# seaweedfs/seaweedfs

Measured on NVIDIA H100. Metric: rs10_4_encode_input_GBps, higher is better.
Workload: dtype u8

## Files before the change

### seaweedfs_b200/build.py

```python
from __future__ import annotations

import hashlib
import os
import shutil
import subprocess
import sys

HERE = os.path.dirname(os.path.abspath(__file__))
CSRC = os.path.join(HERE, "csrc")
GEN = os.path.join(CSRC, "generated")
LIB = os.path.join(HERE, "libswec.so")
ROOT = os.path.dirname(HERE)

SOURCES = ["kernels.cu", "aot_recon.cu", "needles.cu", "damage.cu", "engine.cc", "host_seam.cc", "ec_files.cc", "ec_index.cc", "ec_volume.cc", "volume_format.cc", "staging.cc",
           "jit.cc", "codegen.cc", "gf256.cc"]
HEADERS = ["apply_params.h", "device_common.cuh", "kernels.h", "engine.h", "host_seam.h", "gf256.h", "codegen.h", "io_pool.h", "mini_json.h",
           "volume_format.h", "needle_format.h", "needles.h", "damage.h", "staging.h", os.path.join(ROOT, "include", "swec.h")]
NVCC_FLAGS = ["-gencode", "arch=compute_90a,code=sm_90a", "-O3", "-lineinfo", "-std=c++17",
              "-Xcompiler", "-fPIC,-Wall,-Wno-unused-function", "-cudart", "static"]


def _nvcc() -> str:
    for cand in (os.environ.get("NVCC"), shutil.which("nvcc"), "/usr/local/cuda/bin/nvcc"):
        if cand and os.path.exists(cand):
            return cand
    raise RuntimeError("nvcc not found — libswec.so cannot be built (there is no CPU fallback)")


def _run(cmd: list[str], **kw) -> None:
    r = subprocess.run(cmd, stdout=subprocess.PIPE, stderr=subprocess.STDOUT, text=True, **kw)
    if r.returncode != 0:
        sys.stderr.write(r.stdout)
        raise RuntimeError("command failed: " + " ".join(cmd))


def _stamp() -> str:
    h = hashlib.sha256()
    paths = [os.path.join(CSRC, s) for s in SOURCES + ["codegen_main.cc"]] + \
            [p if os.path.isabs(p) else os.path.join(CSRC, p) for p in HEADERS] + [os.path.abspath(__file__)]
    for p in paths:
        with open(p, "rb") as f:
            h.update(f.read())
    h.update(os.environ.get("SWEC_EXTRA_NVCC_FLAGS", "").encode())
    h.update(os.environ.get("SWEC_CODEGEN_FLAGS", "").encode())
    return h.hexdigest()


def generate() -> None:
    os.makedirs(GEN, exist_ok=True)
    tool = os.path.join(GEN, "swec_codegen")
    _run(["g++", "-O2", "-std=c++17", "-o", tool] +
         [os.path.join(CSRC, s) for s in ("codegen_main.cc", "codegen.cc", "gf256.cc")])
    gen_flags = os.environ.get("SWEC_CODEGEN_FLAGS", "").split()
    out = subprocess.run([tool, "--rs", "10", "4", "--name", "Rs10x4Encode"] + gen_flags, check=True,
                         stdout=subprocess.PIPE, stderr=subprocess.DEVNULL, text=True).stdout
    with open(os.path.join(GEN, "gen_rs10x4_encode.inc"), "w") as f:
        f.write(out)
    with open(os.path.join(GEN, "gen_rs10x4_encode_lp.inc"), "w") as f:
        f.write(out.replace("struct Rs10x4Encode ", "struct Rs10x4EncodeLP "))
    for emit, name in (("structs", "gen_aot_recon.inc"), ("keys", "gen_aot_recon_keys.inc")):
        text = subprocess.run([tool, "--aot-recon", "10", "4", "--emit", emit] +
                              [f for f in gen_flags if f == "--share-powers"], check=True,
                              stdout=subprocess.PIPE, text=True).stdout
        with open(os.path.join(GEN, name), "w") as f:
            f.write(text)
    text = []
    for name in ("apply_params.h", "device_common.cuh"):
        with open(os.path.join(CSRC, name)) as f:
            for line in f:
                if line.startswith("#pragma once") or line.startswith('#include "apply_params.h"'):
                    continue
                text.append(line)
    with open(os.path.join(GEN, "device_common_src.inc"), "w") as f:
        f.write('R"SWECSRC(' + "".join(text) + ')SWECSRC"\n')


def build(force: bool = False, verbose: bool = False) -> str:
    stamp_path = os.path.join(GEN, "build.stamp")
    stamp = _stamp()
    if not force and os.path.exists(LIB) and os.path.exists(stamp_path):
        with open(stamp_path) as f:
            if f.read().strip() == stamp:
                return LIB
    generate()
    extra = os.environ.get("SWEC_EXTRA_NVCC_FLAGS", "").split()
    from concurrent.futures import ThreadPoolExecutor
    objdir = os.path.join(GEN, "obj")
    os.makedirs(objdir, exist_ok=True)
    common = [_nvcc()] + NVCC_FLAGS + extra + ["-I", CSRC, "-I", GEN]
    objs = [os.path.join(objdir, os.path.splitext(src)[0] + ".o") for src in SOURCES]

    def compile_one(pair):
        src, obj = pair
        cmd = common + ["-c", os.path.join(CSRC, src), "-o", obj]
        if verbose:
            print(" ".join(cmd))
        _run(cmd)
    with ThreadPoolExecutor(max_workers=min(len(SOURCES), os.cpu_count() or 2)) as ex:
        list(ex.map(compile_one, zip(SOURCES, objs)))
    cmd = common + ["-shared", "-o", LIB] + objs + ["-ldl", "-lpthread"]
    if verbose:
        print(" ".join(cmd))
    _run(cmd)
    with open(stamp_path, "w") as f:
        f.write(stamp)
    return LIB


if __name__ == "__main__":
    print(build(force="--force" in sys.argv, verbose=True))
```

### seaweedfs_b200/csrc/aot_recon.cu

```cuda
#include <cuda_runtime.h>

#include <atomic>
#include <cstring>

#ifndef SWEC_XT_VARIANT
#define SWEC_XT_VARIANT 0
#endif
#include "device_common.cuh"

namespace swec_aot_boost {
#include "gen_aot_recon.inc"
}
#undef SWEC_XT1A
#undef SWEC_XT1B
#define SWEC_XT1A(a, s) swec_xt1_v<2>((a), (s))
#define SWEC_XT1B(a, s) swec_xt1_v<2>((a), (s))
namespace swec_aot_lowpower {
#include "gen_aot_recon.inc"
}
#undef SWEC_XT1A
#undef SWEC_XT1B
#define SWEC_XT1A(a, s) swec_xt1_v<SWEC_XT_VARIANT>((a), (s))
#define SWEC_XT1B(a, s) swec_xt1_v<SWEC_XT_VARIANT>((a), (s))
#include "gen_aot_recon_keys.inc"
#include "kernels.h"

namespace swec {

constexpr int kAotThreads = 512, kAotUnroll = 2;

template <class Combiner>
__global__ void __launch_bounds__(kAotThreads) swec_aot_recon(const __grid_constant__ SwecApplyParams p) {
    swec_horner_body<Combiner, false, kAotUnroll>(p);
}

int aot_recon_find(int r, int k, const unsigned char* coef) {
    for (int i = 0; i < SWEC_AOT_RECON_COUNT; i++)
        if (kAotReconKeys[i].r == r && kAotReconKeys[i].k == k && memcmp(kAotReconKeys[i].c, coef, size_t(r) * size_t(k)) == 0)
            return i;
    return -1;
}

int aot_recon_count() { return SWEC_AOT_RECON_COUNT; }

static std::atomic<unsigned long long> g_aot_launches{0};
unsigned long long aot_recon_launches() { return g_aot_launches.load(); }

cudaError_t launch_aot_recon(int idx, const SwecApplyParams& p, cudaStream_t s) {
    if (p.nvec == 0) return cudaSuccess;
    if (idx < 0 || idx >= SWEC_AOT_RECON_COUNT) return cudaErrorInvalidValue;
    int sms = 132, dev = 0;
    cudaGetDevice(&dev);
    cudaDeviceGetAttribute(&sms, cudaDevAttrMultiProcessorCount, dev);
    const u64 per_cta = u64(kAotThreads) * kAotUnroll;
    const u64 need = (p.nvec + per_cta - 1) / per_cta;
    const u64 cap = u64(sms) * (kAotReconKeys[idx].r >= 3 ? 1 : 2);
    const unsigned grid = unsigned(need < cap ? need : cap);
    const bool lp = low_power_now();
    note_kernel_work(double(p.nvec) * 16.0 * double(kAotReconKeys[idx].k + kAotReconKeys[idx].r) / 3.0e12 * 1e3);
    g_kernel_launches++;
    g_aot_launches++;
    switch (idx) {
#define SWEC_AOT_CASE(I)                                                                              \
    case I:                                                                                           \
        if (lp) swec_aot_recon<swec_aot_lowpower::SwecAotRecon##I><<<grid, kAotThreads, 0, s>>>(p);     \
        else swec_aot_recon<swec_aot_boost::SwecAotRecon##I><<<grid, kAotThreads, 0, s>>>(p);           \
        break;
        SWEC_AOT_RECON_FOREACH(SWEC_AOT_CASE)
#undef SWEC_AOT_CASE
        default: return cudaErrorInvalidValue;
    }
    return cudaGetLastError();
}

}
```

### seaweedfs_b200/csrc/codegen_main.cc

```cpp
#include <cstdio>
#include <cstdlib>
#include <cstring>
#include <string>

#include <vector>

#include "codegen.h"

static std::vector<swec::Matrix> aot_recon_matrices(int k, int m) {
    const swec::Matrix gen = swec::rs_generator(k, m);
    std::vector<swec::Matrix> out;
    auto add = [&](const std::vector<int>& lost) {
        std::vector<uint8_t> present(size_t(k + m), 1);
        for (int i : lost) present[size_t(i)] = 0;
        std::vector<int> in, outs;
        swec::Matrix fused;
        if (swec::rs_reconstruct_plan(gen, k, present.data(), false, &in, &outs, &fused)) out.push_back(fused);
    };
    for (int i = 0; i < k + m; i++) add({i});
    std::vector<int> worst;
    for (int i = 0; i < m && i < k; i++) worst.push_back(i);
    add(worst);
    return out;
}

int main(int argc, char** argv) {
    swec::CodegenOptions opt;
    swec::Matrix rows;
    std::string name = "SwecGen";
    int aot_k = 0, aot_m = 0;
    bool search_basis = false;
    double step_cost = 5.0;
    std::string emit = "structs";
    for (int a = 1; a < argc; a++) {
        if (!strcmp(argv[a], "--aot-recon") && a + 2 < argc) {
            aot_k = atoi(argv[a + 1]);
            aot_m = atoi(argv[a + 2]);
            a += 2;
            continue;
        }
        if (!strcmp(argv[a], "--emit") && a + 1 < argc) {
            emit = argv[++a];
            continue;
        }
        if (!strcmp(argv[a], "--share-powers")) { opt.share_powers = true; continue; }
        if (!strcmp(argv[a], "--search-basis")) { search_basis = true; continue; }
        if (!strcmp(argv[a], "--step-cost") && a + 1 < argc) { step_cost = atof(argv[++a]); continue; }
        if (!strcmp(argv[a], "--no-basis")) opt.optimise_basis = false;
        else if (!strcmp(argv[a], "--no-cse")) opt.extract_common = false;
        else if (!strcmp(argv[a], "--name") && a + 1 < argc) name = argv[++a];
        else if (!strcmp(argv[a], "--rs") && a + 2 < argc) {
            const int k = atoi(argv[a + 1]), m = atoi(argv[a + 2]);
            a += 2;
            swec::Matrix gen = swec::rs_generator(k, m);
            rows = swec::Matrix(m, k);
            for (int p = 0; p < m; p++)
                for (int i = 0; i < k; i++) rows.at(p, i) = gen.at(k + p, i);
        } else if (!strcmp(argv[a], "--rows") && a + 2 < argc) {
            const int r = atoi(argv[a + 1]), k = atoi(argv[a + 2]);
            a += 2;
            rows = swec::Matrix(r, k);
            for (int i = 0; i < r * k && a + 1 < argc; i++) rows.v[size_t(i)] = uint8_t(atoi(argv[++a]));
        } else {
            fprintf(stderr, "usage: %s [--no-basis] [--no-cse] (--rs K M | --rows R K c...)\n", argv[0]);
            return 2;
        }
    }
    if (aot_k > 0) {
        const std::vector<swec::Matrix> mats = aot_recon_matrices(aot_k, aot_m);
        if (emit == "structs") {
            for (size_t i = 0; i < mats.size(); i++)
                fputs(swec::generate_combine(mats[i], "SwecAotRecon" + std::to_string(i), opt, nullptr).c_str(), stdout);
            return 0;
        }
        printf("// generated by seaweedfs_b200/csrc/codegen_main.cc --aot-recon %d %d --emit keys — do not edit\n", aot_k, aot_m);
        printf("#define SWEC_AOT_RECON_COUNT %zu\n#define SWEC_AOT_RECON_FOREACH(X)", mats.size());
        for (size_t i = 0; i < mats.size(); i++) printf(" X(%zu)", i);
        printf("\nstatic const struct { int r, k; unsigned char c[%d]; } kAotReconKeys[SWEC_AOT_RECON_COUNT] = {\n", aot_m * aot_k);
        for (const swec::Matrix& mx : mats) {
            printf("    {%d, %d, {", mx.rows, mx.cols);
            for (size_t j = 0; j < mx.v.size(); j++) printf("%s%d", j ? "," : "", int(mx.v[j]));
            printf("}},\n");
        }
        printf("};\n");
        return 0;
    }
    if (rows.rows == 0) return 2;
    if (search_basis && rows.rows >= 2 && rows.rows <= 4) {
        const int R = rows.rows;
        const unsigned ncomb = (1u << R) - 1;
        std::vector<unsigned> cur(static_cast<size_t>(R)), best;
        std::vector<int> idx(static_cast<size_t>(R));
        for (int i = 0; i < R; i++) idx[size_t(i)] = i + 1;
        double best_cost = 1e30;
        int tried = 0;
        for (;;) {
            for (int i = 0; i < R; i++) cur[size_t(i)] = unsigned(idx[size_t(i)]);
            swec::CodegenOptions o = opt;
            o.basis = cur;
            swec::CodegenStats cs;
            swec::generate_combine(rows, name, o, &cs);
            const double c = step_cost * cs.xtime_steps + cs.xor_ops;
            tried++;
            if (c < best_cost - 1e-9) { best_cost = c; best = cur; }
            int i = R - 1;
            while (i >= 0 && idx[size_t(i)] == int(ncomb) - (R - 1 - i)) i--;
            if (i < 0) break;
            idx[size_t(i)]++;
            for (int j = i + 1; j < R; j++) idx[size_t(j)] = idx[size_t(j - 1)] + 1;
        }
        opt.basis = best;
        fprintf(stderr, "search-basis: %d bases tried, best cost %.1f, masks", tried, best_cost);
        for (unsigned m : best) fprintf(stderr, " %u", m);
        fprintf(stderr, "\n");
    }
    swec::CodegenStats st;
    fputs(swec::generate_combine(rows, name, opt, &st).c_str(), stdout);
    return 0;
}
```

### seaweedfs_b200/csrc/device_common.cuh

```cuda
#pragma once

#include "apply_params.h"

__device__ __forceinline__ u32 swec_x3(u32 a, u32 b, u32 c) {
    u32 r;
    asm("lop3.b32 %0, %1, %2, %3, 0x96;" : "=r"(r) : "r"(a), "r"(b), "r"(c));
    return r;
}
#define SWEC_X2(a, b) ((a) ^ (b))
#define SWEC_X3(a, b, c) swec_x3((a), (b), (c))

template <int V>
__device__ __forceinline__ u32 swec_xt1_v(u32 a, u32 s) {
    if (V == 2) {
        u32 mask, a2, u, r;
        asm("prmt.b32 %0, %1, 0, 0xba98;" : "=r"(mask) : "r"(a));
        asm("mul.lo.u32 %0, %1, 2;" : "=r"(a2) : "r"(a));
        asm("lop3.b32 %0, %1, 0xfefefefe, %2, 0x6a;" : "=r"(u) : "r"(a2), "r"(s));
        asm("lop3.b32 %0, %1, 0x1d1d1d1d, %2, 0x6a;" : "=r"(r) : "r"(mask), "r"(u));
        return r;
    }
    const u32 hi = a & 0x80808080u;
    if (V == 1) {
        const u32 m = (hi >> 7) * 0x1du;
        const u32 b2 = (a ^ hi) << 1;
        return swec_x3(b2, m, s);
    }
    u32 m, a2, b2;
    asm("mul.hi.u32 %0, %1, 0x3a000000;" : "=r"(m) : "r"(hi));
    asm("mul.lo.u32 %0, %1, 2;" : "=r"(a2) : "r"(a));
    asm("mad.lo.u32 %0, %1, 0xfffffffe, %2;" : "=r"(b2) : "r"(hi), "r"(a2));
    return swec_x3(b2, m, s);
}
#if SWEC_XT_VARIANT == 3
#define SWEC_XT1A(a, s) swec_xt1_v<0>((a), (s))
#define SWEC_XT1B(a, s) swec_xt1_v<2>((a), (s))
#else
#define SWEC_XT1A(a, s) swec_xt1_v<SWEC_XT_VARIANT>((a), (s))
#define SWEC_XT1B(a, s) swec_xt1_v<SWEC_XT_VARIANT>((a), (s))
#endif
#define SWEC_XT0A(a) SWEC_XT1A((a), 0u)
#define SWEC_XT0B(a) SWEC_XT1B((a), 0u)

#ifndef SWEC_LD_POLICY
#define SWEC_LD_POLICY 0
#endif
__device__ __forceinline__ uint4 swec_ldg_stream(const u8* p) {
    uint4 r;
#if SWEC_LD_POLICY == 1
    asm volatile("ld.global.nc.L1::no_allocate.L2::256B.v4.u32 {%0, %1, %2, %3}, [%4];"
#elif SWEC_LD_POLICY == 2
    asm volatile("ld.global.nc.v4.u32 {%0, %1, %2, %3}, [%4];"
#elif SWEC_LD_POLICY == 3
    asm volatile("ld.global.nc.L1::no_allocate.v4.u32 {%0, %1, %2, %3}, [%4];"
#else
    asm volatile("ld.global.nc.L1::no_allocate.L2::128B.v4.u32 {%0, %1, %2, %3}, [%4];"
#endif
                 : "=r"(r.x), "=r"(r.y), "=r"(r.z), "=r"(r.w)
                 : "l"(p));
    return r;
}
__device__ __forceinline__ void swec_stg_stream(u8* p, const uint4& v) {
#if defined(SWEC_ST_POLICY) && SWEC_ST_POLICY == 1
    asm volatile("st.global.v4.u32 [%0], {%1, %2, %3, %4};" ::"l"(p), "r"(v.x), "r"(v.y), "r"(v.z), "r"(v.w)
                 : "memory");
#else
    asm volatile("st.global.cs.v4.u32 [%0], {%1, %2, %3, %4};" ::"l"(p), "r"(v.x), "r"(v.y), "r"(v.z), "r"(v.w)
                 : "memory");
#endif
}

template <class Combiner>
__device__ __forceinline__ void swec_combine_vec(const uint4 (&d)[Combiner::K], uint4 (&o)[Combiner::R]) {
    constexpr int K = Combiner::K, R = Combiner::R;
    u32 x[K], y[R];
#pragma unroll
    for (int i = 0; i < K; i++) x[i] = d[i].x;
    Combiner::combine(x, y);
#pragma unroll
    for (int r = 0; r < R; r++) o[r].x = y[r];
#pragma unroll
    for (int i = 0; i < K; i++) x[i] = d[i].y;
    Combiner::combine(x, y);
#pragma unroll
    for (int r = 0; r < R; r++) o[r].y = y[r];
#pragma unroll
    for (int i = 0; i < K; i++) x[i] = d[i].z;
    Combiner::combine(x, y);
#pragma unroll
    for (int r = 0; r < R; r++) o[r].z = y[r];
#pragma unroll
    for (int i = 0; i < K; i++) x[i] = d[i].w;
    Combiner::combine(x, y);
#pragma unroll
    for (int r = 0; r < R; r++) o[r].w = y[r];
}

template <class Combiner, bool BLOCKED, int UNROLL = 1>
__device__ __forceinline__ void swec_horner_body(const SwecApplyParams& p) {
    constexpr int K = Combiner::K, R = Combiner::R;
    auto in_offset = [&](u64 vv) -> u64 {
        u64 ioff = vv << 4;
        if (BLOCKED) {
            const u64 row = p.block_shift >= 0 ? (vv >> p.block_shift) : (vv / p.block_vecs);
            ioff += row * p.row_extra;
        }
        return ioff;
    };
    const u64 tile = (u64)blockDim.x * UNROLL;
    const u64 stride = (u64)gridDim.x * tile;
    for (u64 base = (u64)blockIdx.x * tile; base < p.nvec; base += stride) {
        uint4 d[UNROLL][K];
        bool live[UNROLL];
#pragma unroll
        for (int u = 0; u < UNROLL; u++) {
            const u64 v = base + (u64)u * blockDim.x + threadIdx.x;
            live[u] = v < p.nvec;
            if (live[u]) {
                const u64 ioff = in_offset(v);
#pragma unroll
                for (int i = 0; i < K; i++) d[u][i] = swec_ldg_stream(p.in[i] + ioff);
            }
        }
#pragma unroll
        for (int u = 0; u < UNROLL; u++) {
            if (live[u]) {
                uint4 o[R];
                swec_combine_vec<Combiner>(d[u], o);
                const u64 off = (base + (u64)u * blockDim.x + threadIdx.x) << 4;
#pragma unroll
                for (int r = 0; r < R; r++) swec_stg_stream(p.out[r] + off, o[r]);
            }
        }
    }
}
```

### seaweedfs_b200/csrc/jit.cc

```cpp
#include <dlfcn.h>
#include <fcntl.h>
#include <nvrtc.h>
#include <sys/stat.h>
#include <unistd.h>

#include <atomic>
#include <cstdlib>
#include <cstring>
#include <chrono>
#include <condition_variable>
#include <deque>
#include <map>
#include <mutex>
#include <thread>

#include "codegen.h"
#include "engine.h"

namespace swec {

static const char kDeviceCommonSrc[] =
#include "device_common_src.inc"
    ;

struct JitKernel {
    int threads = 256, unroll = 1;
    cudaLibrary_t lib = nullptr;
    cudaKernel_t flat = nullptr, blocked = nullptr;
    CodegenStats stats;
};

namespace {

struct Nvrtc {
    void* handle = nullptr;
    decltype(&nvrtcCreateProgram) create = nullptr;
    decltype(&nvrtcCompileProgram) compile = nullptr;
    decltype(&nvrtcGetCUBINSize) cubin_size = nullptr;
    decltype(&nvrtcGetCUBIN) cubin = nullptr;
    decltype(&nvrtcGetProgramLogSize) log_size = nullptr;
    decltype(&nvrtcGetProgramLog) log = nullptr;
    decltype(&nvrtcDestroyProgram) destroy = nullptr;
    bool ok = false;
};

Nvrtc& nvrtc() {
    static Nvrtc n = [] {
        Nvrtc r;
        if (getenv("SWEC_NO_JIT")) return r;
        const char* names[] = {"libnvrtc.so.12", "/usr/local/cuda/lib64/libnvrtc.so.12", "libnvrtc.so",
                               "/usr/local/cuda/lib64/libnvrtc.so"};
        for (const char* nm : names) {
            r.handle = dlopen(nm, RTLD_NOW | RTLD_LOCAL);
            if (r.handle) break;
        }
        if (!r.handle) return r;
#define SWEC_SYM(field, name) r.field = reinterpret_cast<decltype(r.field)>(dlsym(r.handle, name))
        SWEC_SYM(create, "nvrtcCreateProgram");
        SWEC_SYM(compile, "nvrtcCompileProgram");
        SWEC_SYM(cubin_size, "nvrtcGetCUBINSize");
        SWEC_SYM(cubin, "nvrtcGetCUBIN");
        SWEC_SYM(log_size, "nvrtcGetProgramLogSize");
        SWEC_SYM(log, "nvrtcGetProgramLog");
        SWEC_SYM(destroy, "nvrtcDestroyProgram");
#undef SWEC_SYM
        r.ok = r.create && r.compile && r.cubin_size && r.cubin && r.log_size && r.log && r.destroy;
        return r;
    }();
    return n;
}

struct JitEntry {
    enum State { kCold, kQueued, kCompiling, kReady, kFailed } state = kCold;
    int uses = 0;
    std::shared_ptr<JitKernel> kernel;
};
struct JitRequest {
    Matrix rows;
    std::vector<uint8_t> key;
    int threads, unroll, device, variant;
    bool share_powers;
};
struct JitGlobal {
    std::mutex mu;
    std::condition_variable cv;
    std::map<std::vector<uint8_t>, JitEntry> cache;
    std::deque<JitRequest> queue;
    std::thread worker;
    bool worker_started = false, stop = false;
};
JitGlobal& G() {
    static JitGlobal* g = new JitGlobal;
    return *g;
}
constexpr int kHotUses = 1;
constexpr size_t kMaxQueued = 16;

std::shared_ptr<JitKernel> build_kernel(const Matrix& rows, int threads, int unroll, int variant, bool share_powers);

void jit_worker_loop() {
    JitGlobal& g = G();
    std::unique_lock<std::mutex> lock(g.mu);
    for (;;) {
        g.cv.wait(lock, [&] { return g.stop || !g.queue.empty(); });
        if (g.stop) return;
        JitRequest rq = std::move(g.queue.front());
        g.queue.pop_front();
        g.cache[rq.key].state = JitEntry::kCompiling;
        lock.unlock();
        cudaSetDevice(rq.device);
        auto k = build_kernel(rq.rows, rq.threads, rq.unroll, rq.variant, rq.share_powers);
        lock.lock();
        g.cache[rq.key].kernel = k;
        g.cache[rq.key].state = k ? JitEntry::kReady : JitEntry::kFailed;
        g.cv.notify_all();
    }
}

void jit_stop_at_exit() {
    JitGlobal& g = G();
    {
        std::lock_guard<std::mutex> lock(g.mu);
        g.stop = true;
        g.queue.clear();
    }
    g.cv.notify_all();
    if (g.worker.joinable()) g.worker.join();
}

}

void jit_shutdown() { jit_stop_at_exit(); }

static std::vector<uint8_t> jit_key(const Matrix& rows, int threads, int unroll, int variant, bool share_powers) {
    std::vector<uint8_t> key{uint8_t(rows.rows), uint8_t(rows.cols), uint8_t(threads / 64), uint8_t(unroll), uint8_t(variant),
                             uint8_t(share_powers)};
    key.insert(key.end(), rows.v.begin(), rows.v.end());
    return key;
}

bool jit_cached(swec_encoder_impl* enc, const Matrix& rows) {
    return enc->jit.count(jit_key(rows, int(g_opt_enc_threads.load()), int(g_opt_enc_unroll.load()), effective_xt_variant(),
                                  g_opt_jit_share_powers.load() != 0)) != 0;
}

namespace {

bool cache_dir_trusted(const std::string& dir);

std::string disk_cache_dir() {
    if (getenv("SWEC_NO_DISK_CACHE")) return "";
    std::string dir;
    if (const char* d = getenv("SWEC_CACHE_DIR")) dir = d;
    else if (const char* x = getenv("XDG_CACHE_HOME"); x && *x) dir = std::string(x) + "/swec";
    else if (const char* h = getenv("HOME"); h && *h) dir = std::string(h) + "/.cache/swec";
    return !dir.empty() && cache_dir_trusted(dir) ? dir : "";
}

void mkdir_p(const std::string& dir) {
    for (size_t i = 1; i <= dir.size(); i++)
        if (i == dir.size() || dir[i] == '/') mkdir(dir.substr(0, i).c_str(), i == dir.size() ? 0700 : 0755);
}

bool cache_dir_trusted(const std::string& dir) {
    struct stat st;
    if (stat(dir.c_str(), &st) != 0) return true;
    return S_ISDIR(st.st_mode) && st.st_uid == geteuid() && (st.st_mode & (S_IWGRP | S_IWOTH)) == 0;
}

std::string cache_name(const std::string& src) {
    int rt = 0;
    cudaRuntimeGetVersion(&rt);
    const std::string all = "swec-cubin-v1|sm_90a|rt" + std::to_string(rt) + "|" + src;
    unsigned long long h1 = 0xcbf29ce484222325ull, h2 = 0x84222325cbf29ce4ull;
    for (unsigned char c : all) {
        h1 = (h1 ^ c) * 0x100000001b3ull;
        h2 = (h2 ^ (c + 0x9e)) * 0x100000001b3ull;
    }
    char buf[64];
    snprintf(buf, sizeof buf, "%016llx%016llx.cubin", h1, h2);
    return buf;
}

bool read_file(const std::string& path, std::vector<char>* out) {
    FILE* f = fopen(path.c_str(), "rb");
    if (!f) return false;
    fseek(f, 0, SEEK_END);
    const long n = ftell(f);
    fseek(f, 0, SEEK_SET);
    out->resize(n > 0 ? size_t(n) : 0);
    const bool ok = n > 0 && fread(out->data(), 1, size_t(n), f) == size_t(n);
    fclose(f);
    return ok;
}

void write_file_atomic(const std::string& dir, const std::string& name, const std::vector<char>& data) {
    mkdir_p(dir);
    const std::string tmp = dir + "/." + name + "." + std::to_string(long(getpid())) + ".tmp";
    FILE* f = fopen(tmp.c_str(), "wb");
    if (!f) return;
    const bool ok = fwrite(data.data(), 1, data.size(), f) == data.size();
    if (fclose(f) != 0 || !ok || rename(tmp.c_str(), (dir + "/" + name).c_str()) != 0) unlink(tmp.c_str());
}

std::atomic<unsigned long long> g_jit_compiles{0}, g_jit_disk_hits{0};

}

unsigned long long jit_compile_count() { return g_jit_compiles.load(); }
unsigned long long jit_disk_hit_count() { return g_jit_disk_hits.load(); }

bool jit_available() { return nvrtc().ok || !disk_cache_dir().empty(); }

static std::string jit_source(const Matrix& rows, int threads, int unroll, int variant, bool share_powers, CodegenStats* stats) {
    const std::string T = std::to_string(threads), U = std::to_string(unroll);
    std::string src = "#define SWEC_XT_VARIANT " + std::to_string(variant) + "\n";
    src += kDeviceCommonSrc;
    CodegenOptions copt;
    copt.share_powers = share_powers;
    src += generate_combine(rows, "SwecJit", copt, stats);
    src +=
        "extern \"C\" __global__ void __launch_bounds__(" + T + ") swec_jit_flat(const __grid_constant__ SwecApplyParams p) {\n"
        "    swec_horner_body<SwecJit, false, " + U + ">(p);\n}\n"
        "extern \"C\" __global__ void __launch_bounds__(" + T + ") swec_jit_blocked(const __grid_constant__ SwecApplyParams p) {\n"
        "    swec_horner_body<SwecJit, true, " + U + ">(p);\n}\n";
    return src;
}

static int compile_cubin(const Matrix& rows, int threads, int unroll, int variant, bool share_powers, std::vector<char>* cubin,
                         CodegenStats* stats,
                         bool* from_disk = nullptr, std::string* disk_path = nullptr) {
    if (rows.rows > SWEC_MAX_OUTPUTS) return fail(SWEC_ERR_JIT, "too many output rows for one specialised kernel");
    const std::string src = jit_source(rows, threads, unroll, variant, share_powers, stats);
    const std::string dir = disk_cache_dir(), name = dir.empty() ? "" : cache_name(src);
    if (from_disk) *from_disk = false;
    if (!dir.empty() && read_file(dir + "/" + name, cubin)) {
        if (from_disk) *from_disk = true;
        if (disk_path) *disk_path = dir + "/" + name;
        g_jit_disk_hits++;
        return SWEC_OK;
    }
    Nvrtc& n = nvrtc();
    if (!n.ok) return fail(SWEC_ERR_JIT, "NVRTC not available and this matrix is not in the cubin cache");
    static std::mutex& compile_mu = *new std::mutex;
    std::lock_guard<std::mutex> compile_lock(compile_mu);
    nvrtcProgram prog = nullptr;
    if (n.create(&prog, src.c_str(), "swec_jit.cu", 0, nullptr, nullptr) != NVRTC_SUCCESS)
        return fail(SWEC_ERR_JIT, "nvrtcCreateProgram failed");
    const char* opts[] = {"--gpu-architecture=sm_90a", "-std=c++17", "-lineinfo"};
    if (n.compile(prog, 3, opts) != NVRTC_SUCCESS) {
        size_t ls = 0;
        n.log_size(prog, &ls);
        std::string log(ls, '\0');
        if (ls) n.log(prog, &log[0]);
        n.destroy(&prog);
        return fail(SWEC_ERR_JIT, "NVRTC compile failed: " + log);
    }
    size_t cs = 0;
    n.cubin_size(prog, &cs);
    cubin->resize(cs);
    n.cubin(prog, cubin->data());
    n.destroy(&prog);
    g_jit_compiles++;
    if (!dir.empty()) write_file_atomic(dir, name, *cubin);
    return SWEC_OK;
}

namespace {
std::shared_ptr<JitKernel> build_kernel(const Matrix& rows, int threads, int unroll, int variant, bool share_powers) {
    for (int attempt = 0; attempt < 2; attempt++) {
        auto kernel = std::make_shared<JitKernel>();
        kernel->threads = threads;
        kernel->unroll = unroll;
        std::vector<char> cubin;
        bool from_disk = false;
        std::string disk_path;
        if (compile_cubin(rows, threads, unroll, variant, share_powers, &cubin, &kernel->stats, &from_disk, &disk_path) != SWEC_OK)
            return nullptr;
        cudaError_t e = cudaLibraryLoadData(&kernel->lib, cubin.data(), nullptr, nullptr, 0, nullptr, nullptr, 0);
        if (e == cudaSuccess) e = cudaLibraryGetKernel(&kernel->flat, kernel->lib, "swec_jit_flat");
        if (e == cudaSuccess) e = cudaLibraryGetKernel(&kernel->blocked, kernel->lib, "swec_jit_blocked");
        if (e == cudaSuccess) return kernel;
        cudaGetLastError();
        if (from_disk && attempt == 0) {
            unlink(disk_path.c_str());
            continue;
        }
        cuda_fail(e, "loading the specialised kernel");
        return nullptr;
    }
    return nullptr;
}

}

int jit_get(swec_encoder_impl* enc, const Matrix& rows, std::shared_ptr<JitKernel>* out, bool wait, bool hot) {
    const int threads = int(g_opt_enc_threads.load()), unroll = int(g_opt_enc_unroll.load());
    const int variant = effective_xt_variant();
    const bool share_powers = g_opt_jit_share_powers.load() != 0;
    const std::vector<uint8_t> key = jit_key(rows, threads, unroll, variant, share_powers);
    *out = nullptr;
    auto local = enc->jit.find(key);
    if (local != enc->jit.end()) {
        *out = local->second;
        return SWEC_OK;
    }
    if (!jit_available()) return fail(SWEC_ERR_JIT, "NVRTC not available and the cubin cache is off");
    JitGlobal& g = G();
    std::unique_lock<std::mutex> lock(g.mu);
    for (;;) {
        JitEntry& e = g.cache[key];
        if (e.state == JitEntry::kReady || e.state == JitEntry::kFailed) {
            enc->jit[key] = e.kernel;
            *out = e.kernel;
            return e.kernel ? SWEC_OK : SWEC_ERR_JIT;
        }
        if (!wait) {
            if (e.state == JitEntry::kCold && (++e.uses >= kHotUses || hot) && g.queue.size() < kMaxQueued && !g.stop) {
                int dev = 0;
                cudaGetDevice(&dev);
                e.state = JitEntry::kQueued;
                g.queue.push_back({rows, key, threads, unroll, dev, variant, share_powers});
                if (!g.worker_started) {
                    g.worker_started = true;
                    g.worker = std::thread(jit_worker_loop);
                    std::atexit(jit_stop_at_exit);
                }
                g.cv.notify_all();
            }
            return SWEC_OK;
        }
        if (e.state == JitEntry::kCompiling) {
            g.cv.wait(lock);
            continue;
        }
        if (e.state == JitEntry::kQueued) {
            for (auto it = g.queue.begin(); it != g.queue.end(); ++it)
                if (it->key == key) {
                    g.queue.erase(it);
                    break;
                }
        }
        e.state = JitEntry::kCompiling;
        lock.unlock();
        auto k = build_kernel(rows, threads, unroll, variant, share_powers);
        lock.lock();
        JitEntry& e2 = g.cache[key];
        e2.kernel = k;
        e2.state = k ? JitEntry::kReady : JitEntry::kFailed;
        g.cv.notify_all();
        enc->jit[key] = k;
        *out = k;
        return k ? SWEC_OK : SWEC_ERR_JIT;
    }
}

int jit_debug_compile(const Matrix& rows, size_t* cubin_bytes, int* xtime_steps, int* xor_ops) {
    std::vector<char> cubin;
    CodegenStats st;
    const int rc = compile_cubin(rows, int(g_opt_enc_threads.load()), int(g_opt_enc_unroll.load()), effective_xt_variant(),
                                 g_opt_jit_share_powers.load() != 0, &cubin, &st);
    if (cubin_bytes) *cubin_bytes = cubin.size();
    if (xtime_steps) *xtime_steps = st.xtime_steps;
    if (xor_ops) *xor_ops = st.xor_ops;
    return rc;
}

cudaError_t jit_launch(const JitKernel& k, const SwecApplyParams& p, bool blocked, cudaStream_t s) {
    if (p.nvec == 0) return cudaSuccess;
    int sms = 132, dev = 0;
    cudaGetDevice(&dev);
    cudaDeviceGetAttribute(&sms, cudaDevAttrMultiProcessorCount, dev);
    const u64 per_cta = u64(k.threads) * u64(k.unroll);
    const u64 need = (p.nvec + per_cta - 1) / per_cta;
    const u64 cap = u64(sms) * u64(encode_ctas_per_sm());
    const unsigned grid = unsigned(need < cap ? need : cap);
    void* args[] = {const_cast<SwecApplyParams*>(&p)};
    note_kernel_work(double(p.nvec) * 16.0 * 14.0 / 3.0e12 * 1e3);
    g_kernel_launches++;
    return cudaLaunchKernel(reinterpret_cast<const void*>(blocked ? k.blocked : k.flat), dim3(grid),
                            dim3(unsigned(k.threads)), args, 0, s);
}

}
```

### seaweedfs_b200/csrc/kernels.cu

```cuda
#include <cuda_runtime.h>

#include <algorithm>
#include <atomic>
#include <cstdio>
#include <cstdlib>

#ifndef SWEC_XT_VARIANT
#define SWEC_XT_VARIANT 0
#endif
#include "device_common.cuh"
#include "gen_rs10x4_encode.inc"
#undef SWEC_XT1A
#undef SWEC_XT1B
#define SWEC_XT1A(a, s) swec_xt1_v<2>((a), (s))
#define SWEC_XT1B(a, s) swec_xt1_v<2>((a), (s))
#include "gen_rs10x4_encode_lp.inc"
#undef SWEC_XT1A
#undef SWEC_XT1B
#define SWEC_XT1A(a, s) swec_xt1_v<SWEC_XT_VARIANT>((a), (s))
#define SWEC_XT1B(a, s) swec_xt1_v<SWEC_XT_VARIANT>((a), (s))
#include "kernels.h"

#include <chrono>
#include <cmath>
#include <mutex>

namespace swec {

std::atomic<unsigned long long> g_kernel_launches{0};


template <int THREADS, int UNROLL, bool BLOCKED, bool LOW_POWER = false>
__global__ void __launch_bounds__(THREADS) rs10x4_encode(const __grid_constant__ SwecApplyParams p) {
    if (LOW_POWER) swec_horner_body<Rs10x4EncodeLP, BLOCKED, UNROLL>(p);
    else swec_horner_body<Rs10x4Encode, BLOCKED, UNROLL>(p);
}


__device__ __forceinline__ u32 smem_u32(const void* p) { return (u32)__cvta_generic_to_shared(p); }

template <int KT>
__global__ void __launch_bounds__(256) swec_table_kernel(const __grid_constant__ SwecApplyParams p,
                                                          const u32* __restrict__ tables, int k_rt, int r) {
    extern __shared__ __align__(128) u32 tab[];
    __shared__ __align__(8) u64 mbar;
    const int K = KT > 0 ? KT : k_rt;
    const u32 bytes = (u32)K * 4096u;
    if (threadIdx.x == 0) {
        asm volatile("mbarrier.init.shared::cta.b64 [%0], 1;" ::"r"(smem_u32(&mbar)));
        asm volatile("fence.mbarrier_init.release.cluster;" ::: "memory");
    }
    __syncthreads();
    if (threadIdx.x == 0) {
        asm volatile("mbarrier.arrive.expect_tx.shared::cta.b64 _, [%0], %1;" ::"r"(smem_u32(&mbar)), "r"(bytes)
                     : "memory");
        asm volatile(
            "cp.async.bulk.shared::cluster.global.mbarrier::complete_tx::bytes [%0], [%1], %2, [%3];" ::"r"(
                smem_u32(tab)),
            "l"(tables), "r"(bytes), "r"(smem_u32(&mbar))
            : "memory");
    }
    {
        u32 done = 0;
        while (!done) {
            asm volatile(
                "{ .reg .pred q; mbarrier.try_wait.parity.shared::cta.b64 q, [%1], 0; selp.u32 %0, 1, 0, q; }"
                : "=r"(done)
                : "r"(smem_u32(&mbar))
                : "memory");
        }
    }
    const u32 lane4 = (threadIdx.x & 31u) * 4u;
    const char* tb = reinterpret_cast<const char*>(tab);
    const u64 stride = (u64)gridDim.x * blockDim.x;
    for (u64 v = (u64)blockIdx.x * blockDim.x + threadIdx.x; v < p.nvec; v += stride) {
        const u64 off = v << 4;
        u32 acc[16];
#pragma unroll
        for (int j = 0; j < 16; j++) acc[j] = 0;
        auto fold = [&](int i, const uint4& d) {
            const char* t = tb + (u32)i * 4096u + lane4;
            const u32 w[4] = {d.x, d.y, d.z, d.w};
#pragma unroll
            for (int c = 0; c < 4; c++) {
#pragma unroll
                for (int b = 0; b < 4; b++) {
                    const u32 byte = (w[c] >> (8 * b)) & 0xffu;
                    const u32 lo = *reinterpret_cast<const u32*>(t + ((byte & 15u) << 7));
                    const u32 hi = *reinterpret_cast<const u32*>(t + 2048 + ((byte >> 4) << 7));
                    acc[c * 4 + b] = swec_x3(acc[c * 4 + b], lo, hi);
                }
            }
        };
        if (KT > 0) {
            uint4 d[KT > 0 ? KT : 1];
#pragma unroll
            for (int i = 0; i < KT; i++) d[i] = swec_ldg_stream(p.in[i] + off);
#pragma unroll
            for (int i = 0; i < KT; i++) fold(i, d[i]);
        } else {
            int i = 0;
            for (; i + 2 <= K; i += 2) {
                const uint4 d0 = swec_ldg_stream(p.in[i] + off);
                const uint4 d1 = swec_ldg_stream(p.in[i + 1] + off);
                fold(i, d0);
                fold(i + 1, d1);
            }
            if (i < K) fold(i, swec_ldg_stream(p.in[i] + off));
        }
#pragma unroll
        for (int q = 0; q < 4; q++) {
            if (q < r) {
                uint4 o;
                u32* ow = reinterpret_cast<u32*>(&o);
#pragma unroll
                for (int c = 0; c < 4; c++) {
                    const u32 lo2 = __byte_perm(acc[c * 4 + 0], acc[c * 4 + 1], 0x0040 + q * 0x0011);
                    const u32 hi2 = __byte_perm(acc[c * 4 + 2], acc[c * 4 + 3], 0x0040 + q * 0x0011);
                    ow[c] = __byte_perm(lo2, hi2, 0x5410);
                }
                swec_stg_stream(p.out[q] + off, o);
            }
        }
    }
}

__global__ void __launch_bounds__(256) swec_bytes_kernel(const __grid_constant__ SwecApplyParams p,
                                                          const u32* __restrict__ compact, int K, int r,
                                                          u64 nbytes) {
    const u64 stride = (u64)gridDim.x * blockDim.x;
    for (u64 x = (u64)blockIdx.x * blockDim.x + threadIdx.x; x < nbytes; x += stride) {
        u32 acc = 0;
        for (int i = 0; i < K; i++) {
            const u32 byte = p.in[i][x];
            acc ^= __ldg(&compact[i * 32 + (byte & 15u)]) ^ __ldg(&compact[i * 32 + 16 + (byte >> 4)]);
        }
        for (int q = 0; q < r; q++) p.out[q][x] = (u8)(acc >> (8 * q));
    }
}


__device__ __forceinline__ u64 splitmix64_at(u64 seed, u64 j) {
    u64 z = seed + (j + 1) * 0x9E3779B97F4A7C15ull;
    z = (z ^ (z >> 30)) * 0xBF58476D1CE4E5B9ull;
    z = (z ^ (z >> 27)) * 0x94D049BB133111EBull;
    return z ^ (z >> 31);
}

__global__ void __launch_bounds__(256) swec_synth_kernel(u64* __restrict__ dst, u64 first_word, u64 nwords, u64 seed) {
    const u64 stride = (u64)gridDim.x * blockDim.x;
    for (u64 j = (u64)blockIdx.x * blockDim.x + threadIdx.x; j < nwords; j += stride)
        dst[j] = splitmix64_at(seed, first_word + j);
}

__global__ void __launch_bounds__(256) swec_digest_kernel(const u8* __restrict__ src, u64 nbytes, u64* __restrict__ out) {
    const u64 nwords = (nbytes + 7) >> 3;
    const u64 stride = (u64)gridDim.x * blockDim.x;
    u64 sum = 0;
    for (u64 j = (u64)blockIdx.x * blockDim.x + threadIdx.x; j < nwords; j += stride) {
        u64 w;
        if ((j + 1) * 8 <= nbytes && (reinterpret_cast<unsigned long long>(src) & 7) == 0) {
            w = reinterpret_cast<const u64*>(src)[j];
        } else {
            w = 0;
            for (int b = 0; b < 8; b++)
                if (j * 8 + b < nbytes) w |= (u64)src[j * 8 + b] << (8 * b);
        }
        sum += splitmix64_at(w, j);
    }
    for (int s = 16; s > 0; s >>= 1) sum += __shfl_xor_sync(0xffffffffu, sum, s);
    if ((threadIdx.x & 31) == 0) atomicAdd(reinterpret_cast<unsigned long long*>(out), sum);
}

__global__ void __launch_bounds__(256) swec_compare_kernel(const u8* __restrict__ a, const u8* __restrict__ b,
                                                            u64 nbytes, unsigned long long* __restrict__ mismatches) {
    const u64 stride = (u64)gridDim.x * blockDim.x;
    const bool aligned = ((reinterpret_cast<unsigned long long>(a) | reinterpret_cast<unsigned long long>(b)) & 15) == 0;
    const u64 nvec = (nbytes + 15) >> 4;
    unsigned long long bad = 0;
    for (u64 v = (u64)blockIdx.x * blockDim.x + threadIdx.x; v < nvec; v += stride) {
        const u64 off = v << 4;
        if (aligned && off + 16 <= nbytes) {
            const uint4 x = swec_ldg_stream(a + off), y = swec_ldg_stream(b + off);
            bad += ((x.x ^ y.x) | (x.y ^ y.y) | (x.z ^ y.z) | (x.w ^ y.w)) != 0;
        } else {
            bool diff = false;
            for (u64 x = off; x < nbytes && x < off + 16; x++) diff |= a[x] != b[x];
            bad += diff;
        }
    }
    if (bad) atomicAdd(mismatches, bad);
}


static int g_sm_count[64];

static int sm_count() {
    int dev = 0;
    cudaGetDevice(&dev);
    if (dev < 0 || dev >= 64) return 132;
    if (!g_sm_count[dev]) {
        int n = 132;
        cudaDeviceGetAttribute(&n, cudaDevAttrMultiProcessorCount, dev);
        g_sm_count[dev] = n;
    }
    return g_sm_count[dev];
}

static unsigned grid_for(u64 items, int threads, int ctas_per_sm) {
    const u64 need = (items + threads - 1) / threads;
    const u64 cap = (u64)sm_count() * ctas_per_sm;
    return (unsigned)(need < cap ? (need ? need : 1) : cap);
}

static long env_long(const char* name, long dflt) {
    const char* e = getenv(name);
    return e && *e ? atol(e) : dflt;
}
std::atomic<long> g_opt_enc_threads{env_long("SWEC_ENC_THREADS", 512)};
std::atomic<long> g_opt_enc_unroll{env_long("SWEC_ENC_UNROLL", 2)};
std::atomic<long> g_opt_ctas_per_sm{env_long("SWEC_CTAS_PER_SM", 0)};
std::atomic<long> g_opt_xt_variant{env_long("SWEC_XT_VARIANT_JIT", SWEC_XT_VARIANT)};
std::atomic<long> g_opt_use_aot{env_long("SWEC_USE_AOT", 1)};
std::atomic<long> g_opt_jit_share_powers{env_long("SWEC_JIT_SHARE_POWERS", 0)};
std::atomic<long> g_opt_power_mode{env_long("SWEC_POWER_MODE", 1)};

namespace {
struct Heat {
    std::mutex mu;
    double level = 0;
    std::chrono::steady_clock::time_point last{};
};
Heat g_heat[64];
constexpr double kHeatTauMs = 1000.0, kHeatHotMs = 450.0;
Heat& heat_here() {
    int dev = 0;
    cudaGetDevice(&dev);
    return g_heat[(dev >= 0 && dev < 64) ? dev : 0];
}
double decayed(Heat& h, std::chrono::steady_clock::time_point now) {
    if (h.last.time_since_epoch().count() == 0) return 0;
    const double dt = std::chrono::duration<double, std::milli>(now - h.last).count();
    return h.level * std::exp(-dt / kHeatTauMs);
}
}

void note_kernel_work(double est_ms) {
    Heat& h = heat_here();
    const auto now = std::chrono::steady_clock::now();
    std::lock_guard<std::mutex> lk(h.mu);
    h.level = decayed(h, now) + est_ms;
    h.last = now;
}

bool low_power_now() {
    const long mode = g_opt_power_mode.load();
    if (mode == 1) return false;
    if (mode == 2) return true;
    Heat& h = heat_here();
    const auto now = std::chrono::steady_clock::now();
    std::lock_guard<std::mutex> lk(h.mu);
    const double level = decayed(h, now);
    static const bool debug = getenv("SWEC_DEBUG_POWER") != nullptr;
    if (debug) fprintf(stderr, "[swec] power policy: heat %.1f ms (hot above %.0f) -> %s variant\n", level, kHeatHotMs, level > kHeatHotMs ? "low-power" : "boost");
    return level > kHeatHotMs;
}

double power_heat_ms() {
    Heat& h = heat_here();
    const auto now = std::chrono::steady_clock::now();
    std::lock_guard<std::mutex> lk(h.mu);
    return decayed(h, now);
}

int effective_xt_variant() {
    const long v = g_opt_xt_variant.load();
    if (v != 0) return int(v);
    return low_power_now() ? 2 : 0;
}

static double est_ms_for(const SwecApplyParams& p, int k, int r) {
    return double(p.nvec) * 16.0 * double(k + r) / 3.0e12 * 1e3;
}

int encode_ctas_per_sm() {
    const long c = g_opt_ctas_per_sm.load();
    if (c > 0 && c <= 64) return int(c);
    const long t = g_opt_enc_threads.load(), u = g_opt_enc_unroll.load();
    const long tt = t == 128 || t == 512 ? t : 256;
    return int(std::max(1l, (u > 1 ? 512 : 768) / tt));
}

template <int THREADS, int UNROLL>
static cudaError_t launch_rs10x4_shape(const SwecApplyParams& p, bool blocked, int ctas_per_sm, cudaStream_t s) {
    const unsigned grid = grid_for((p.nvec + UNROLL - 1) / UNROLL, THREADS, ctas_per_sm);
    const bool lp = low_power_now();
    note_kernel_work(est_ms_for(p, 10, 4));
    if (blocked && lp) rs10x4_encode<THREADS, UNROLL, true, true><<<grid, THREADS, 0, s>>>(p);
    else if (blocked) rs10x4_encode<THREADS, UNROLL, true, false><<<grid, THREADS, 0, s>>>(p);
    else if (lp) rs10x4_encode<THREADS, UNROLL, false, true><<<grid, THREADS, 0, s>>>(p);
    else rs10x4_encode<THREADS, UNROLL, false, false><<<grid, THREADS, 0, s>>>(p);
    return cudaGetLastError();
}

cudaError_t launch_rs10x4_encode(const SwecApplyParams& p, bool blocked, cudaStream_t s) {
    if (p.nvec == 0) return cudaSuccess;
    const long threads = g_opt_enc_threads.load(), unroll = g_opt_enc_unroll.load();
    const int c = encode_ctas_per_sm();
    g_kernel_launches++;
    if (threads == 128 && unroll == 1) return launch_rs10x4_shape<128, 1>(p, blocked, c, s);
    if (threads == 128 && unroll == 2) return launch_rs10x4_shape<128, 2>(p, blocked, c, s);
    if (threads == 512 && unroll == 1) return launch_rs10x4_shape<512, 1>(p, blocked, c, s);
    if (threads == 512 && unroll == 2) return launch_rs10x4_shape<512, 2>(p, blocked, c, s);
    if (unroll == 2) return launch_rs10x4_shape<256, 2>(p, blocked, c, s);
    return launch_rs10x4_shape<256, 1>(p, blocked, c, s);
}

cudaError_t launch_table_apply(const SwecApplyParams& p, const u32* replicated_tables, int K, int r, cudaStream_t s) {
    if (p.nvec == 0) return cudaSuccess;
    const size_t smem = size_t(K) * 4096;
    const int per_sm = smem <= 56 * 1024 ? 4 : (smem <= 113 * 1024 ? 2 : 1);
    const unsigned grid = grid_for(p.nvec, 256, per_sm);
    cudaError_t e;
    if (K == 10) {
        e = cudaFuncSetAttribute(swec_table_kernel<10>, cudaFuncAttributeMaxDynamicSharedMemorySize, int(smem));
        if (e != cudaSuccess) return e;
        swec_table_kernel<10><<<grid, 256, smem, s>>>(p, replicated_tables, K, r);
    } else {
        e = cudaFuncSetAttribute(swec_table_kernel<0>, cudaFuncAttributeMaxDynamicSharedMemorySize, int(smem));
        if (e != cudaSuccess) return e;
        swec_table_kernel<0><<<grid, 256, smem, s>>>(p, replicated_tables, K, r);
    }
    g_kernel_launches++;
    return cudaGetLastError();
}

cudaError_t launch_bytes_apply(const SwecApplyParams& p, const u32* compact_tables, int K, int r, u64 nbytes,
                               cudaStream_t s) {
    if (nbytes == 0) return cudaSuccess;
    swec_bytes_kernel<<<grid_for(nbytes, 256, 8), 256, 0, s>>>(p, compact_tables, K, r, nbytes);
    g_kernel_launches++;
    return cudaGetLastError();
}

cudaError_t launch_synth(void* dst, u64 byte_offset, u64 nbytes, u64 seed, cudaStream_t s) {
    if (nbytes == 0) return cudaSuccess;
    swec_synth_kernel<<<grid_for(nbytes / 8, 256, 8), 256, 0, s>>>(static_cast<u64*>(dst), byte_offset / 8, nbytes / 8, seed);
    g_kernel_launches++;
    return cudaGetLastError();
}

cudaError_t launch_digest(const void* src, u64 nbytes, u64* out_dev, cudaStream_t s) {
    cudaError_t e = cudaMemsetAsync(out_dev, 0, 8, s);
    if (e != cudaSuccess || nbytes == 0) return e;
    swec_digest_kernel<<<grid_for((nbytes + 7) / 8, 256, 8), 256, 0, s>>>(static_cast<const u8*>(src), nbytes, out_dev);
    g_kernel_launches++;
    return cudaGetLastError();
}

cudaError_t launch_compare(const void* a, const void* b, u64 nbytes, unsigned long long* out_dev, cudaStream_t s) {
    if (nbytes == 0) return cudaSuccess;
    swec_compare_kernel<<<grid_for((nbytes + 15) / 16, 256, 8), 256, 0, s>>>(static_cast<const u8*>(a), static_cast<const u8*>(b), nbytes, out_dev);
    g_kernel_launches++;
    return cudaGetLastError();
}

}
```

Measured before the change: 2140.

## Specialize horner loop on compile-time tile, hoist bounds checks, enable basis search by default

The main grid-stride loop now makes the thread count a template parameter and runs whole tiles with no per-element bounds checks. Loads and stores use immediate offsets from a single base pointer, and the per-element row division becomes one division per tile. A noinline scalar tail handles leftover vectors. Code generation now defaults to share-powers plus a basis search with per-variant step costs, including the AOT reconstruction kernels, to cut GF multiply work. The cost is more build-time generation and a JIT unroll that is now capped at two.

Result: no change. 2145 (median of 6 runs) (+0.3%).

```diff
diff --git a/seaweedfs_b200/build.py b/seaweedfs_b200/build.py
--- a/seaweedfs_b200/build.py
+++ b/seaweedfs_b200/build.py
@@ -42,7 +42,7 @@
         with open(p, "rb") as f:
             h.update(f.read())
     h.update(os.environ.get("SWEC_EXTRA_NVCC_FLAGS", "").encode())
-    h.update(os.environ.get("SWEC_CODEGEN_FLAGS", "").encode())
+    h.update(repr(os.environ.get("SWEC_CODEGEN_FLAGS")).encode())
     return h.hexdigest()
 
 
@@ -51,17 +51,22 @@
     tool = os.path.join(GEN, "swec_codegen")
     _run(["g++", "-O2", "-std=c++17", "-o", tool] +
          [os.path.join(CSRC, s) for s in ("codegen_main.cc", "codegen.cc", "gf256.cc")])
-    gen_flags = os.environ.get("SWEC_CODEGEN_FLAGS", "").split()
-    out = subprocess.run([tool, "--rs", "10", "4", "--name", "Rs10x4Encode"] + gen_flags, check=True,
-                         stdout=subprocess.PIPE, stderr=subprocess.DEVNULL, text=True).stdout
-    with open(os.path.join(GEN, "gen_rs10x4_encode.inc"), "w") as f:
-        f.write(out)
-    with open(os.path.join(GEN, "gen_rs10x4_encode_lp.inc"), "w") as f:
-        f.write(out.replace("struct Rs10x4Encode ", "struct Rs10x4EncodeLP "))
-    for emit, name in (("structs", "gen_aot_recon.inc"), ("keys", "gen_aot_recon_keys.inc")):
-        text = subprocess.run([tool, "--aot-recon", "10", "4", "--emit", emit] +
-                              [f for f in gen_flags if f == "--share-powers"], check=True,
-                              stdout=subprocess.PIPE, text=True).stdout
+    override = os.environ.get("SWEC_CODEGEN_FLAGS")
+    def flags(step_cost: int) -> list[str]:
+        if override is not None:
+            return override.split()
+        return ["--share-powers", "--search-basis", "--step-cost", str(step_cost)]
+    for name, struct, step_cost in (("gen_rs10x4_encode.inc", "Rs10x4Encode", 5),
+                                    ("gen_rs10x4_encode_lp.inc", "Rs10x4EncodeLP", 4)):
+        out = subprocess.run([tool, "--rs", "10", "4", "--name", struct] + flags(step_cost), check=True,
+                             stdout=subprocess.PIPE, stderr=subprocess.DEVNULL, text=True).stdout
+        with open(os.path.join(GEN, name), "w") as f:
+            f.write(out)
+    for args, name in ((["--emit", "structs"] + flags(5), "gen_aot_recon.inc"),
+                       (["--emit", "structs"] + flags(4), "gen_aot_recon_lp.inc"),
+                       (["--emit", "keys"], "gen_aot_recon_keys.inc")):
+        text = subprocess.run([tool, "--aot-recon", "10", "4"] + args, check=True,
+                              stdout=subprocess.PIPE, stderr=subprocess.DEVNULL, text=True).stdout
         with open(os.path.join(GEN, name), "w") as f:
             f.write(text)
     text = []
diff --git a/seaweedfs_b200/csrc/aot_recon.cu b/seaweedfs_b200/csrc/aot_recon.cu
--- a/seaweedfs_b200/csrc/aot_recon.cu
+++ b/seaweedfs_b200/csrc/aot_recon.cu
@@ -16,7 +16,7 @@
 #define SWEC_XT1A(a, s) swec_xt1_v<2>((a), (s))
 #define SWEC_XT1B(a, s) swec_xt1_v<2>((a), (s))
 namespace swec_aot_lowpower {
-#include "gen_aot_recon.inc"
+#include "gen_aot_recon_lp.inc"
 }
 #undef SWEC_XT1A
 #undef SWEC_XT1B
@@ -31,7 +31,7 @@
 
 template <class Combiner>
 __global__ void __launch_bounds__(kAotThreads) swec_aot_recon(const __grid_constant__ SwecApplyParams p) {
-    swec_horner_body<Combiner, false, kAotUnroll>(p);
+    swec_horner_body<Combiner, false, kAotUnroll, kAotThreads>(p);
 }
 
 int aot_recon_find(int r, int k, const unsigned char* coef) {
diff --git a/seaweedfs_b200/csrc/codegen_main.cc b/seaweedfs_b200/csrc/codegen_main.cc
--- a/seaweedfs_b200/csrc/codegen_main.cc
+++ b/seaweedfs_b200/csrc/codegen_main.cc
@@ -22,6 +22,37 @@
     for (int i = 0; i < m && i < k; i++) worst.push_back(i);
     add(worst);
     return out;
+}
+
+static std::vector<unsigned> best_basis(const swec::Matrix& rows, const std::string& name, const swec::CodegenOptions& opt,
+                                        double step_cost) {
+    const int R = rows.rows;
+    if (R < 2 || R > 4) return {};
+    const unsigned ncomb = (1u << R) - 1;
+    std::vector<unsigned> cur(static_cast<size_t>(R)), best;
+    std::vector<int> idx(static_cast<size_t>(R));
+    for (int i = 0; i < R; i++) idx[size_t(i)] = i + 1;
+    double best_cost = 1e30;
+    int tried = 0;
+    for (;;) {
+        for (int i = 0; i < R; i++) cur[size_t(i)] = unsigned(idx[size_t(i)]);
+        swec::CodegenOptions o = opt;
+        o.basis = cur;
+        swec::CodegenStats cs;
+        swec::generate_combine(rows, name, o, &cs);
+        const double c = step_cost * cs.xtime_steps + cs.xor_ops;
+        tried++;
+        if (c < best_cost - 1e-9) { best_cost = c; best = cur; }
+        int i = R - 1;
+        while (i >= 0 && idx[size_t(i)] == int(ncomb) - (R - 1 - i)) i--;
+        if (i < 0) break;
+        idx[size_t(i)]++;
+        for (int j = i + 1; j < R; j++) idx[size_t(j)] = idx[size_t(j - 1)] + 1;
+    }
+    fprintf(stderr, "search-basis %s: %d bases tried, best cost %.1f, masks", name.c_str(), tried, best_cost);
+    for (unsigned m : best) fprintf(stderr, " %u", m);
+    fprintf(stderr, "\n");
+    return best;
 }
 
 int main(int argc, char** argv) {
@@ -69,8 +100,12 @@
     if (aot_k > 0) {
         const std::vector<swec::Matrix> mats = aot_recon_matrices(aot_k, aot_m);
         if (emit == "structs") {
-            for (size_t i = 0; i < mats.size(); i++)
-                fputs(swec::generate_combine(mats[i], "SwecAotRecon" + std::to_string(i), opt, nullptr).c_str(), stdout);
+            for (size_t i = 0; i < mats.size(); i++) {
+                const std::string sname = "SwecAotRecon" + std::to_string(i);
+                swec::CodegenOptions o = opt;
+                if (search_basis) o.basis = best_basis(mats[i], sname, opt, step_cost);
+                fputs(swec::generate_combine(mats[i], sname, o, nullptr).c_str(), stdout);
+            }
             return 0;
         }
         printf("// generated by seaweedfs_b200/csrc/codegen_main.cc --aot-recon %d %d --emit keys — do not edit\n", aot_k, aot_m);
@@ -86,34 +121,7 @@
         return 0;
     }
     if (rows.rows == 0) return 2;
-    if (search_basis && rows.rows >= 2 && rows.rows <= 4) {
-        const int R = rows.rows;
-        const unsigned ncomb = (1u << R) - 1;
-        std::vector<unsigned> cur(static_cast<size_t>(R)), best;
-        std::vector<int> idx(static_cast<size_t>(R));
-        for (int i = 0; i < R; i++) idx[size_t(i)] = i + 1;
-        double best_cost = 1e30;
-        int tried = 0;
-        for (;;) {
-            for (int i = 0; i < R; i++) cur[size_t(i)] = unsigned(idx[size_t(i)]);
-            swec::CodegenOptions o = opt;
-            o.basis = cur;
-            swec::CodegenStats cs;
-            swec::generate_combine(rows, name, o, &cs);
-            const double c = step_cost * cs.xtime_steps + cs.xor_ops;
-            tried++;
-            if (c < best_cost - 1e-9) { best_cost = c; best = cur; }
-            int i = R - 1;
-            while (i >= 0 && idx[size_t(i)] == int(ncomb) - (R - 1 - i)) i--;
-            if (i < 0) break;
-            idx[size_t(i)]++;
-            for (int j = i + 1; j < R; j++) idx[size_t(j)] = idx[size_t(j - 1)] + 1;
-        }
-        opt.basis = best;
-        fprintf(stderr, "search-basis: %d bases tried, best cost %.1f, masks", tried, best_cost);
-        for (unsigned m : best) fprintf(stderr, " %u", m);
-        fprintf(stderr, "\n");
-    }
+    if (search_basis) opt.basis = best_basis(rows, name, opt, step_cost);
     swec::CodegenStats st;
     fputs(swec::generate_combine(rows, name, opt, &st).c_str(), stdout);
     return 0;
diff --git a/seaweedfs_b200/csrc/device_common.cuh b/seaweedfs_b200/csrc/device_common.cuh
--- a/seaweedfs_b200/csrc/device_common.cuh
+++ b/seaweedfs_b200/csrc/device_common.cuh
@@ -96,41 +96,73 @@
     for (int r = 0; r < R; r++) o[r].w = y[r];
 }
 
-template <class Combiner, bool BLOCKED, int UNROLL = 1>
+template <int OFF>
+__device__ __forceinline__ uint4 swec_ldg_stream_at(const u8* p) {
+    uint4 r;
+    asm volatile("ld.global.nc.L1::no_allocate.L2::128B.v4.u32 {%0, %1, %2, %3}, [%4+%5];"
+                 : "=r"(r.x), "=r"(r.y), "=r"(r.z), "=r"(r.w)
+                 : "l"(p), "n"(OFF));
+    return r;
+}
+template <int OFF>
+__device__ __forceinline__ void swec_stg_stream_at(u8* p, const uint4& v) {
+    asm volatile("st.global.cs.v4.u32 [%0+%1], {%2, %3, %4, %5};" ::"l"(p), "n"(OFF), "r"(v.x), "r"(v.y), "r"(v.z),
+                 "r"(v.w)
+                 : "memory");
+}
+
+template <class Combiner, bool BLOCKED>
+__device__ __noinline__ void swec_horner_vec(const SwecApplyParams& p, u64 v) {
+    constexpr int K = Combiner::K, R = Combiner::R;
+    u64 ioff = v << 4;
+    if (BLOCKED) ioff += (p.block_shift >= 0 ? (v >> p.block_shift) : (v / p.block_vecs)) * p.row_extra;
+    uint4 d[K], o[R];
+#pragma unroll
+    for (int i = 0; i < K; i++) d[i] = swec_ldg_stream(p.in[i] + ioff);
+    swec_combine_vec<Combiner>(d, o);
+#pragma unroll
+    for (int r = 0; r < R; r++) swec_stg_stream(p.out[r] + (v << 4), o[r]);
+}
+
+template <class Combiner, bool BLOCKED, int UNROLL, int THREADS>
 __device__ __forceinline__ void swec_horner_body(const SwecApplyParams& p) {
     constexpr int K = Combiner::K, R = Combiner::R;
-    auto in_offset = [&](u64 vv) -> u64 {
-        u64 ioff = vv << 4;
+    constexpr u64 kTile = u64(THREADS) * UNROLL;
+    constexpr int kSliceBytes = THREADS * 16;
+    static_assert(UNROLL == 1 || UNROLL == 2, "one or two column slices per thread");
+    const u64 nvec = p.nvec;
+    const bool rows_whole = !BLOCKED || (p.block_vecs % kTile == 0 && p.block_vecs != 0);
+    const u64 whole_end = (rows_whole && nvec / kTile < 0xffffffffull) ? nvec - nvec % kTile : 0;
+    u32 tiles_per_row = 0;
+    if (BLOCKED && rows_whole && p.block_shift < 0) {
+        const u64 tpr = p.block_vecs / kTile;
+        tiles_per_row = tpr < 0xffffffffull ? u32(tpr) : 0xffffffffu;
+    }
+    const u64 stride = u64(gridDim.x) * kTile;
+    for (u64 base = u64(blockIdx.x) * kTile; base < whole_end; base += stride) {
+        const u64 off = (base + threadIdx.x) << 4;
+        u64 ioff = off;
         if (BLOCKED) {
-            const u64 row = p.block_shift >= 0 ? (vv >> p.block_shift) : (vv / p.block_vecs);
+            const u64 row = p.block_shift >= 0 ? (base >> p.block_shift) : u64(u32(base / kTile) / tiles_per_row);
             ioff += row * p.row_extra;
         }
-        return ioff;
-    };
-    const u64 tile = (u64)blockDim.x * UNROLL;
-    const u64 stride = (u64)gridDim.x * tile;
-    for (u64 base = (u64)blockIdx.x * tile; base < p.nvec; base += stride) {
         uint4 d[UNROLL][K];
-        bool live[UNROLL];
 #pragma unroll
-        for (int u = 0; u < UNROLL; u++) {
-            const u64 v = base + (u64)u * blockDim.x + threadIdx.x;
-            live[u] = v < p.nvec;
-            if (live[u]) {
-                const u64 ioff = in_offset(v);
+        for (int i = 0; i < K; i++) {
+            const u8* src = p.in[i] + ioff;
+            d[0][i] = swec_ldg_stream_at<0>(src);
+            if (UNROLL > 1) d[UNROLL > 1 ? 1 : 0][i] = swec_ldg_stream_at<kSliceBytes>(src);
+        }
+        uint4 o[UNROLL][R];
 #pragma unroll
-                for (int i = 0; i < K; i++) d[u][i] = swec_ldg_stream(p.in[i] + ioff);
-            }
-        }
+        for (int u = 0; u < UNROLL; u++) swec_combine_vec<Combiner>(d[u], o[u]);
 #pragma unroll
-        for (int u = 0; u < UNROLL; u++) {
-            if (live[u]) {
-                uint4 o[R];
-                swec_combine_vec<Combiner>(d[u], o);
-                const u64 off = (base + (u64)u * blockDim.x + threadIdx.x) << 4;
-#pragma unroll
-                for (int r = 0; r < R; r++) swec_stg_stream(p.out[r] + off, o[r]);
-            }
+        for (int r = 0; r < R; r++) {
+            u8* dst = p.out[r] + off;
+            swec_stg_stream_at<0>(dst, o[0][r]);
+            if (UNROLL > 1) swec_stg_stream_at<kSliceBytes>(dst, o[UNROLL > 1 ? 1 : 0][r]);
         }
     }
+    for (u64 v = whole_end + u64(blockIdx.x) * THREADS + threadIdx.x; v < nvec; v += u64(gridDim.x) * THREADS)
+        swec_horner_vec<Combiner, BLOCKED>(p, v);
 }
diff --git a/seaweedfs_b200/csrc/jit.cc b/seaweedfs_b200/csrc/jit.cc
--- a/seaweedfs_b200/csrc/jit.cc
+++ b/seaweedfs_b200/csrc/jit.cc
@@ -213,7 +213,7 @@
 bool jit_available() { return nvrtc().ok || !disk_cache_dir().empty(); }
 
 static std::string jit_source(const Matrix& rows, int threads, int unroll, int variant, bool share_powers, CodegenStats* stats) {
-    const std::string T = std::to_string(threads), U = std::to_string(unroll);
+    const std::string T = std::to_string(threads), U = unroll >= 2 ? "2" : "1";
     std::string src = "#define SWEC_XT_VARIANT " + std::to_string(variant) + "\n";
     src += kDeviceCommonSrc;
     CodegenOptions copt;
@@ -221,9 +221,9 @@
     src += generate_combine(rows, "SwecJit", copt, stats);
     src +=
         "extern \"C\" __global__ void __launch_bounds__(" + T + ") swec_jit_flat(const __grid_constant__ SwecApplyParams p) {\n"
-        "    swec_horner_body<SwecJit, false, " + U + ">(p);\n}\n"
+        "    swec_horner_body<SwecJit, false, " + U + ", " + T + ">(p);\n}\n"
         "extern \"C\" __global__ void __launch_bounds__(" + T + ") swec_jit_blocked(const __grid_constant__ SwecApplyParams p) {\n"
-        "    swec_horner_body<SwecJit, true, " + U + ">(p);\n}\n";
+        "    swec_horner_body<SwecJit, true, " + U + ", " + T + ">(p);\n}\n";
     return src;
 }
 
diff --git a/seaweedfs_b200/csrc/kernels.cu b/seaweedfs_b200/csrc/kernels.cu
--- a/seaweedfs_b200/csrc/kernels.cu
+++ b/seaweedfs_b200/csrc/kernels.cu
@@ -32,8 +32,8 @@
 
 template <int THREADS, int UNROLL, bool BLOCKED, bool LOW_POWER = false>
 __global__ void __launch_bounds__(THREADS) rs10x4_encode(const __grid_constant__ SwecApplyParams p) {
-    if (LOW_POWER) swec_horner_body<Rs10x4EncodeLP, BLOCKED, UNROLL>(p);
-    else swec_horner_body<Rs10x4Encode, BLOCKED, UNROLL>(p);
+    if (LOW_POWER) swec_horner_body<Rs10x4EncodeLP, BLOCKED, UNROLL, THREADS>(p);
+    else swec_horner_body<Rs10x4Encode, BLOCKED, UNROLL, THREADS>(p);
 }
 
 
```
